# learnedsystems/RMI

Hardware: NVIDIA H100
Metric: RMI build keys/sec (200M uint64, linear,linear 2^20) (higher is better)
Workload: dtype f64

## Files before the change

### rmi_b200/csrc/api.cu

```cuda
#include <algorithm>
#include <fcntl.h>
#include <sys/mman.h>
#include <unistd.h>
#include <atomic>
#include <chrono>
#include <cstdlib>
#include <cmath>
#include <cstdio>
#include <cstring>
#include <memory>
#include <mutex>
#include <string>
#include <vector>

#include "../../include/rmi_b200.h"
#include "kernels.h"
#include "nccl_dl.h"
#include "../../host/cache_fix.hpp"
#include "../../host/artefact_load.hpp"
#include "../../host/codegen.hpp"
#include "../../host/optimizer.hpp"
#include "../../host/slab_layout.hpp"

using namespace rmi;
// ... 573 lines not shown
    rmihost::output_rmi(ns, *r, data_dir, key_type, include_errors != 0, build_time_ns, out_dir, knots ? &cf : nullptr);
    return RMI_OK;
  } catch (const std::exception& e) {
    return fail(RMI_ERR_PANIC, e.what());
  }
}

int rmi_load_rmi(const char* ns, const char* out_dir, const char* data_dir, rmi_result** out, rmi_spline_point** knots,
                 rmi_artefact_info* info) {
  g_last_error.clear();
  if (!ns || !out_dir || !data_dir || !out || !knots || !info) return fail(RMI_ERR_INVALID, "rmi_load_rmi: null argument");
  auto a = std::make_unique<rmihost::LoadedArtefact>();
  try {
    rmihost::load_rmi(ns, out_dir, data_dir, a.get());
  } catch (const rmihost::LoadError& e) {
    return fail(e.code, e.what());
  } catch (const std::exception& e) {
    return fail(RMI_ERR_INVALID, std::string("rmi_load_rmi: ") + e.what());
  }
  rmi_spline_point* pts = nullptr;
  if (!a->knots.empty()) {
    pts = static_cast<rmi_spline_point*>(std::malloc(a->knots.size() * sizeof(rmi_spline_point)));
    if (!pts) return fail(RMI_ERR_INVALID, "rmi_load_rmi: out of host memory");
    for (size_t k = 0; k < a->knots.size(); ++k) { pts[k].key = a->knots[k].first; pts[k].offset = a->knots[k].second; }
  }
  auto box = new ResultBox();
  box->pub = a->r;
  *out = &box->pub;
  *knots = pts;
  info->key_type = a->key_type;
  info->has_errors = a->has_errors ? 1 : 0;
  info->line_size = a->line_size;
  info->num_knots = a->knots.size();
  info->num_data_rows = a->r.num_data_rows;
  info->build_time_ns = a->build_time_ns;
  box->loaded = std::move(a);
  return RMI_OK;
}

int rmi_find_pareto_efficient_configs(const rmi_dataset* const* replicas, int num_replicas, uint64_t restrict_to,
                                      uint32_t flags, rmi_config_stats* out, uint64_t capacity, uint64_t* out_count) {
  g_last_error.clear();
  if (!replicas || num_replicas < 1 || !out_count || (capacity && !out))
    return fail(RMI_ERR_INVALID, "rmi_find_pareto_efficient_configs: bad argument");
  try {
    std::vector<const rmi_dataset*> reps(replicas, replicas + num_replicas);
    std::vector<rmihost::RMIStatistics> front = rmihost::find_pareto_efficient_configs(reps, (size_t)restrict_to, flags, false);
    *out_count = front.size();
    for (size_t i = 0; i < front.size() && i < capacity; ++i) {
      std::snprintf(out[i].models, sizeof out[i].models, "%s", front[i].models.c_str());
      out[i].branching_factor = front[i].branching_factor;
      out[i].average_log2_error = front[i].average_log2_error;
      out[i].max_log2_error = front[i].max_log2_error;
      out[i].size = front[i].size;
    }
    return RMI_OK;
  } catch (const std::exception& e) {
    return fail(RMI_ERR_PANIC, e.what());
  }
}

int rmi_dataset_replicate(const rmi_dataset* src, int device, rmi_dataset** out) {
  g_last_error.clear();
  if (!src || !out) return fail(RMI_ERR_INVALID, "rmi_dataset_replicate: null argument");
  const size_t ksz = src->key_type == RMI_KEY_U32 ? 4 : 8;
  const size_t bytes = ((size_t)src->n * ksz + 15) & ~(size_t)15;
  CUDA_TRY(cudaSetDevice(device));
  void* d = nullptr;
  CUDA_TRY(cudaMalloc(&d, bytes ? bytes : 16));
  cudaError_t e = cudaSuccess;
  if (src->n) {
    if (device != src->device) {
      int can = 0;
      cudaDeviceCanAccessPeer(&can, device, src->device);
      if (can) { cudaError_t pe = cudaDeviceEnablePeerAccess(src->device, 0); if (pe != cudaSuccess) cudaGetLastError(); }
    }
    e = cudaMemcpyPeer(d, device, src->d_keys, src->device, (size_t)src->n * ksz);
    if (e == cudaSuccess) e = cudaDeviceSynchronize();
  }
  if (e != cudaSuccess) { cudaFree(d); return fail(RMI_ERR_CUDA, std::string("rmi_dataset_replicate: ") + cudaGetErrorString(e)); }
  auto* ds = new rmi_dataset();
  ds->d_keys = d; ds->n = src->n; ds->key_type = src->key_type; ds->device = device;
  ds->owned = true; ds->pooled = false; ds->sorted = src->sorted; ds->no_dups = src->no_dups;
  *out = ds;
  return RMI_OK;
}

uint64_t rmi_dataset_len(const rmi_dataset* ds) { return ds ? ds->n : 0; }
int rmi_dataset_key_type(const rmi_dataset* ds) { return ds ? ds->key_type : -1; }
void rmi_dataset_destroy(rmi_dataset* ds) {
  if (!ds) return;
  if (ds->owned && ds->d_keys) {
    cudaSetDevice(ds->device);
    if (ds->pooled) cudaFreeAsync(ds->d_keys, nullptr); else cudaFree(ds->d_keys);
  }
  delete ds;
}

void rmi_result_free(rmi_result* r) { delete reinterpret_cast<ResultBox*>(r); }

}

struct rmi_index {
  const rmi_dataset* ds = nullptr;
  TopTables tables;
  TopModel top;
  int leaf_kind = 0;
  uint64_t N = 0;
  uint64_t n = 0;
  void* d_records = nullptr;
  int num_sms = 0;
  void* d_knots = nullptr;
  uint64_t K = 0;
  uint64_t line_size = 0;
};

namespace {
void index_free_device(rmi_index* idx) {
  idx->tables.free_device();
  cudaFree(idx->d_records);
  cudaFree(idx->d_knots);
}

int index_check_call(const rmi_index* idx, const void* d_queries, uint64_t n, const void* d_out, const char* fn) {
  if (!idx) return fail(RMI_ERR_INVALID, std::string(fn) + ": null index");
  if (n && (!d_queries || !d_out)) return fail(RMI_ERR_INVALID, std::string(fn) + ": null query or output pointer");
  return RMI_OK;
}

int index_launch(const rmi_index* idx, const void* d_queries, uint64_t n, uint64_t* d_out, uint64_t* d_err,
                 uint64_t* d_fallbacks, void* cuda_stream, bool lower_bound) {
  if (n == 0) return RMI_OK;
  const rmi_dataset* ds = idx->ds;
  CUDA_TRY(cudaSetDevice(ds->device));
  Launch L{(cudaStream_t)cuda_stream, idx->num_sms};
  if (idx->d_knots) {
    lookup_bounded_batch(L, idx->top, idx->leaf_kind, idx->d_records, idx->N, idx->d_knots, idx->K, idx->line_size,
                         (const u64*)ds->d_keys, idx->n, (const u64*)d_queries, n, (u64*)d_out, (u64*)d_err,
                         (u64*)d_fallbacks, lower_bound);
    CUDA_TRY(cudaGetLastError());
    return RMI_OK;
  }
  with_key_type(ds->key_type, [&](auto k) {
    using T = decltype(k);
    lookup_batch<T>(L, idx->top, idx->leaf_kind, idx->d_records, idx->N, (const T*)ds->d_keys, idx->n,
                    (const T*)d_queries, n, (u64*)d_out, (u64*)d_err, (u64*)d_fallbacks, lower_bound);
  });
  CUDA_TRY(cudaGetLastError());
  return RMI_OK;
}
int index_check_tables(const rmi_result* r, uint64_t rows, const char* holder, uint64_t keys, const std::string& fn) {
  if (r->num_rmi_rows != rows)
    return fail(RMI_ERR_INVALID, fn + ": the result was trained on " + std::to_string(r->num_rmi_rows) + " keys, " +
                                     holder + std::to_string(rows));
  if (keys == 0 || r->branching_factor == 0) return fail(RMI_ERR_INVALID, fn + ": empty index");
  return RMI_OK;
}

int index_upload(const rmi_result* r, const rmi_dataset* ds, uint64_t n, const rmi_spline_point* knots, uint64_t K,
                 uint64_t line_size, const std::string& fn, rmi_index** out) {
  CUDA_TRY(cudaSetDevice(ds->device));
  DeviceInfo di;
  if (int rc = device_info(ds->device, &di)) return rc;
  auto* idx = new rmi_index();
  idx->ds = ds;
  idx->leaf_kind = (int)r->l1_model_id;
  idx->N = r->branching_factor;
  idx->n = n;
  idx->num_sms = di.num_sms;
  std::vector<char> packed((size_t)idx->N * lookup_record_bytes(idx->leaf_kind));
  pack_leaf_records(idx->leaf_kind, r->l1_params, (const u64*)r->l1_errors, idx->N, packed.data());
  cudaError_t e = idx->tables.upload(*r, nullptr, device_alloc);
  idx->top = idx->tables.given(*r);
  if (e == cudaSuccess) e = cudaMalloc(&idx->d_records, packed.size());
  if (e == cudaSuccess) e = cudaMemcpy(idx->d_records, packed.data(), packed.size(), cudaMemcpyHostToDevice);
  if (e == cudaSuccess && knots) {
    e = cudaMalloc(&idx->d_knots, sizeof(rmi_spline_point) * K);
    if (e == cudaSuccess) e = cudaMemcpy(idx->d_knots, knots, sizeof(rmi_spline_point) * K, cudaMemcpyHostToDevice);
    idx->K = K;
    idx->line_size = line_size;
  }
  if (e == cudaSuccess) e = cudaStreamSynchronize(nullptr);
  if (e != cudaSuccess) {
    index_free_device(idx);
    delete idx;
    return fail(RMI_ERR_CUDA, fn + ": " + cudaGetErrorString(e));
  }
  *out = idx;
  return RMI_OK;
}


}

extern "C" {

int rmi_index_create(const rmi_result* r, const rmi_dataset* ds, rmi_index** out) {
  const std::string fn = "rmi_index_create";
  if (!r || !ds || !out) return fail(RMI_ERR_INVALID, fn + ": null argument");
  if (int rc = check_result(r, true, fn)) return rc;
  if (int rc = index_check_tables(r, ds->n, "the dataset holds ", ds->n, fn)) return rc;
  return index_upload(r, ds, ds->n, nullptr, 0, 0, fn, out);
}

int rmi_index_create_bounded(const rmi_result* r, const rmi_spline_point* knots, uint64_t num_knots,
                             uint64_t line_size, const rmi_dataset* ds, rmi_index** out) {
  const std::string fn = "rmi_index_create_bounded";
  if (!r || !knots || !ds || !out) return fail(RMI_ERR_INVALID, fn + ": null argument");
  if (int rc = check_result(r, true, fn)) return rc;
  if (ds->key_type != RMI_KEY_U64) return fail(RMI_ERR_INVALID, fn + ": Can only construct a bounded RMI on u64 data");
  if (line_size == 0) return fail(RMI_ERR_INVALID, fn + ": line size 0");
  if (num_knots == 0) return fail(RMI_ERR_INVALID, fn + ": no spline knots");
  if (int rc = index_check_tables(r, num_knots, "the spline has ", ds->n, fn)) return rc;
  for (uint64_t i = 0; i < num_knots; ++i) {
    if (knots[i].offset >= ds->n)
      return fail(RMI_ERR_INVALID, fn + ": knot " + std::to_string(i) + " has offset " + std::to_string(knots[i].offset) +
                                       ", the dataset holds " + std::to_string(ds->n) + " keys");
    if (i && !(knots[i - 1].key < knots[i].key && knots[i - 1].offset <= knots[i].offset))
      return fail(RMI_ERR_INVALID, fn + ": knots " + std::to_string(i - 1) + " and " + std::to_string(i) +
                                       " are out of order (keys must increase strictly, offsets must not decrease)");
  }
  return index_upload(r, ds, ds->n, knots, num_knots, line_size, fn, out);
}

void rmi_index_destroy(rmi_index* idx) {
  if (!idx) return;
  cudaSetDevice(idx->ds->device);
  index_free_device(idx);
  delete idx;
}

int rmi_index_predict(const rmi_index* idx, const void* d_queries, uint64_t n, uint64_t* d_pos, uint64_t* d_err,
                      void* cuda_stream) {
  if (int rc = index_check_call(idx, d_queries, n, d_pos, "rmi_index_predict")) return rc;
  return index_launch(idx, d_queries, n, d_pos, d_err, nullptr, cuda_stream, false);
}

int rmi_index_lower_bound(const rmi_index* idx, const void* d_queries, uint64_t n, uint64_t* d_out,
                          uint64_t* d_fallbacks, void* cuda_stream) {
  if (int rc = index_check_call(idx, d_queries, n, d_out, "rmi_index_lower_bound")) return rc;
  return index_launch(idx, d_queries, n, d_out, nullptr, d_fallbacks, cuda_stream, true);
}

int rmi_index_lookup_host(const rmi_index* idx, const void* host_queries, uint64_t n, int lower_bound,
                          uint64_t* host_out, uint64_t* host_err, uint64_t* fallbacks) {
  if (int rc = index_check_call(idx, host_queries, n, host_out, "rmi_index_lookup_host")) return rc;
  if (n == 0) return RMI_OK;
  CUDA_TRY(cudaSetDevice(idx->ds->device));
  const size_t qb = (size_t)n * key_bytes(idx->ds->key_type), ob = (size_t)n * sizeof(uint64_t);
  cudaStream_t st = nullptr;
  char* d = nullptr;
  cudaError_t e = cudaStreamCreateWithFlags(&st, cudaStreamNonBlocking);
  if (e == cudaSuccess) e = cudaMallocAsync((void**)&d, qb + 2 * ob + 8 + 8, st);
  int rc = RMI_OK;
  if (e == cudaSuccess) {
    char* d_q = d;
    uint64_t* d_out = (uint64_t*)(d + ((qb + 7) & ~(size_t)7));
    uint64_t* d_err = d_out + n;
    uint64_t* d_fb = d_err + n;
    e = cudaMemcpyAsync(d_q, host_queries, qb, cudaMemcpyHostToDevice, st);
    if (e == cudaSuccess) e = cudaMemsetAsync(d_fb, 0, sizeof(u64), st);
    if (e == cudaSuccess) {
      rc = lower_bound ? index_launch(idx, d_q, n, d_out, nullptr, d_fb, st, true)
                       : index_launch(idx, d_q, n, d_out, host_err ? d_err : nullptr, nullptr, st, false);
    }
    if (e == cudaSuccess && rc == RMI_OK) e = cudaMemcpyAsync(host_out, d_out, ob, cudaMemcpyDeviceToHost, st);
    if (e == cudaSuccess && rc == RMI_OK && !lower_bound && host_err)
      e = cudaMemcpyAsync(host_err, d_err, ob, cudaMemcpyDeviceToHost, st);
    if (e == cudaSuccess && rc == RMI_OK && lower_bound && fallbacks)
      e = cudaMemcpyAsync(fallbacks, d_fb, sizeof(u64), cudaMemcpyDeviceToHost, st);
    cudaFreeAsync(d, st);
  }
  if (st) {
    cudaError_t es = cudaStreamSynchronize(st);
    if (e == cudaSuccess) e = es;
    cudaStreamDestroy(st);
  }
  if (rc != RMI_OK) return rc;
  if (e != cudaSuccess) return fail(RMI_ERR_CUDA, std::string("rmi_index_lookup_host: ") + cudaGetErrorString(e));
  return RMI_OK;
}

}

namespace {

struct SliceResources {
  int device = -1;
  LeafCopyOut co;
  void release() {
    if (device < 0) return;
    for (int c = 0; c < LEAF_SLICES; ++c) {
      if (co.streams[c]) cudaStreamDestroy(co.streams[c]);
      if (co.ev_kernel[c]) cudaEventDestroy(co.ev_kernel[c]);
      if (co.ev_copied[c]) cudaEventDestroy(co.ev_copied[c]);
    }
    if (co.ev_ready) cudaEventDestroy(co.ev_ready);
    co = LeafCopyOut();
    device = -1;
  }
  LeafCopyOut* get(int dev) {
    if (device == dev) return &co;
    release();
    bool ok = cudaEventCreateWithFlags(&co.ev_ready, cudaEventDisableTiming) == cudaSuccess;
    for (int c = 0; c < LEAF_SLICES && ok; ++c)
      ok = cudaStreamCreateWithFlags(&co.streams[c], cudaStreamNonBlocking) == cudaSuccess &&
           cudaEventCreateWithFlags(&co.ev_kernel[c], cudaEventDisableTiming) == cudaSuccess &&
           cudaEventCreateWithFlags(&co.ev_copied[c], cudaEventDisableTiming) == cudaSuccess;
    device = dev;
    if (!ok) { release(); cudaGetLastError(); return nullptr; }
    return &co;
  }
  ~SliceResources() {}
};
thread_local SliceResources t_slices;

struct BuildContext {
  int device = -1;
  cudaStream_t st = nullptr, side = nullptr;
  cudaEvent_t ev0 = nullptr, ev1 = nullptr, evp[3] = {nullptr, nullptr, nullptr}, ev_fork = nullptr, ev_join = nullptr;
  void release() {
    if (device < 0) return;
    if (st) cudaStreamDestroy(st);
    if (side) cudaStreamDestroy(side);
    for (cudaEvent_t e : {ev0, ev1, evp[0], evp[1], evp[2], ev_fork, ev_join}) if (e) cudaEventDestroy(e);
    *this = BuildContext();
  }
  BuildContext* get(int dev) {
    if (device == dev) return this;
    release();
    int lo_prio = 0, hi_prio = 0;
    cudaDeviceGetStreamPriorityRange(&lo_prio, &hi_prio);
    bool ok = cudaStreamCreateWithFlags(&st, cudaStreamNonBlocking) == cudaSuccess &&
              cudaEventCreate(&ev0) == cudaSuccess && cudaEventCreate(&ev1) == cudaSuccess &&
              cudaEventCreate(&evp[0]) == cudaSuccess && cudaEventCreate(&evp[1]) == cudaSuccess &&
              cudaEventCreate(&evp[2]) == cudaSuccess &&
              cudaEventCreateWithFlags(&ev_fork, cudaEventDisableTiming) == cudaSuccess &&
              cudaEventCreateWithFlags(&ev_join, cudaEventDisableTiming) == cudaSuccess;
    if (ok && cudaStreamCreateWithPriority(&side, cudaStreamNonBlocking, hi_prio) != cudaSuccess) { side = nullptr; cudaGetLastError(); }
    device = dev;
    if (!ok) { release(); cudaGetLastError(); return nullptr; }
    return this;
  }
};
thread_local BuildContext t_build_ctx;

struct Arena {
  cudaStream_t st;
  std::vector<void*> ptrs;
  cudaError_t err = cudaSuccess;
  explicit Arena(cudaStream_t s) : st(s) {}
  template <class P> P* get(size_t count) {
    void* p = nullptr;
    cudaError_t e = cudaMallocAsync(&p, std::max<size_t>(count * sizeof(P), 16), st);
    if (e != cudaSuccess) { err = e; return nullptr; }
    ptrs.push_back(p);
    return (P*)p;
  }
  ~Arena() { for (void* p : ptrs) cudaFreeAsync(p, st); }
};

template <class T> inline double host_as_float(T k) { return (double)k; }
inline uint64_t host_scale(uint64_t off, double sf, bool use_sf) { return use_sf ? (uint64_t)((double)off * sf) : off; }

template <class T>
unsigned host_exact_top(const rmi_dataset* ds, int kind, uint64_t N, double* out_f) {
  const uint64_t n = ds->n;
  const T* d_keys = (const T*)ds->d_keys;
  const double sf = (double)N / (double)n;
  const bool use_sf = std::fabs(sf - 1.0) > DBL_EPSILON;
  uint64_t i0 = 0, i1 = n;
  bool repeat = true;
  if (kind == M_ROBUST_LINEAR) {
    uint64_t bnd = (uint64_t)((double)n * 0.0001);
    if (bnd < 1) bnd = 1;
    if (!(bnd * 2 + 1 < n)) return ST_ROBUST_TOO_SMALL;
    i0 = bnd; i1 = n - bnd; repeat = false;
  }
  const size_t PIECE = ((size_t)64 << 20) / sizeof(T);
  T* stage[2] = {(T*)g_pinned.get(PIECE * sizeof(T)), (T*)g_pinned.get(PIECE * sizeof(T))};
  cudaStream_t cs = nullptr;
  cudaEvent_t ev[2] = {nullptr, nullptr};
  bool ok = stage[0] && stage[1] && cudaStreamCreateWithFlags(&cs, cudaStreamNonBlocking) == cudaSuccess &&
            cudaEventCreateWithFlags(&ev[0], cudaEventDisableTiming) == cudaSuccess &&
            cudaEventCreateWithFlags(&ev[1], cudaEventDisableTiming) == cudaSuccess;
  unsigned status = 0;
  if (ok) {
    const int passes = kind == M_NORMAL ? 2 : 1;
    double mean_x = 0.0, mean_y = 0.0, c = 0.0, m2 = 0.0;
    uint64_t cnt = 0;
    double nmean = 0.0, nstd = 0.0;
    const double nf = (double)n;
    T last_key = T();
    uint64_t last_F = 0;
    for (int pass = 0; pass < passes && ok; ++pass) {
      auto issue = [&](uint64_t piece) {
        const uint64_t a = piece * PIECE, b = std::min<uint64_t>(n, a + PIECE);
        cudaMemcpyAsync(stage[piece & 1], d_keys + a, (b - a) * sizeof(T), cudaMemcpyDeviceToHost, cs);
        cudaEventRecord(ev[piece & 1], cs);
      };
      const uint64_t npieces = (n + PIECE - 1) / PIECE;
      if (npieces) issue(0);
      uint64_t F = 0;
      T prev = T();
      for (uint64_t piece = 0; piece < npieces && ok; ++piece) {
        if (cudaEventSynchronize(ev[piece & 1]) != cudaSuccess) { ok = false; break; }
        if (piece + 1 < npieces) issue(piece + 1);
        const T* kb = stage[piece & 1];
        const uint64_t a = piece * PIECE, b = std::min<uint64_t>(n, a + PIECE);
        for (uint64_t i = a; i < b; ++i) {
          const T k = kb[i - a];
          if (i == 0 || k != prev) F = i;
          prev = k;
          if (kind == M_NORMAL) {
            const double x = host_as_float(k);
            if (pass == 0) nmean = nmean + x / nf;
            else { const double d = x - nmean; nstd = nstd + d * d; }
          } else if (i >= i0 && i < i1) {
            const double x = host_as_float(k), y = (double)host_scale(F, sf, use_sf);
            cnt += 1;
            const double dx = x - mean_x;
            const double cf = (double)cnt;
            mean_x = mean_x + dx / cf;
            mean_y = mean_y + (y - mean_y) / cf;
            c = c + dx * (y - mean_y);
            const double dx2 = x - mean_x;
            m2 = m2 + dx * dx2;
          }
        }
        if (b == n && n > 0) { last_key = prev; last_F = F; }
      }
      if (!ok) break;
      if (n > 0) {
        const double x = host_as_float(last_key);
        if (kind == M_NORMAL) {
          if (pass == 0) nmean = nmean + x / nf;
          else { const double d = x - nmean; nstd = nstd + d * d; }
        } else if (repeat) {
          const double y = (double)host_scale(last_F, sf, use_sf);
          cnt += 1;
          const double dx = x - mean_x;
          const double cf = (double)cnt;
          mean_x = mean_x + dx / cf;
          mean_y = mean_y + (y - mean_y) / cf;
          c = c + dx * (y - mean_y);
          const double dx2 = x - mean_x;
          m2 = m2 + dx * dx2;
        }
      }
    }
    if (ok) {
      if (kind == M_NORMAL) {
        out_f[0] = nmean;
        out_f[1] = std::sqrt(nstd / nf);
        out_f[2] = n > 0 ? std::fmax(-INFINITY, (double)host_scale(last_F, sf, use_sf)) : -INFINITY;
      } else {
        double alpha, beta;
        if (cnt == 0) { alpha = 0.0; beta = 0.0; }
        else if (cnt == 1) { alpha = mean_y; beta = 0.0; }
        else {
          const double nm1 = (double)(cnt - 1);
          const double cov = c / nm1, var = m2 / nm1;
          if (!(var >= 0.0)) { status |= ST_NEG_VARIANCE; alpha = 0.0; beta = 0.0; }
          else if (var == 0.0) { alpha = mean_y; beta = 0.0; }
          else { beta = cov / var; alpha = mean_y - beta * mean_x; }
        }
        out_f[0] = alpha; out_f[1] = beta;
      }
    }
  }
  if (cs) { cudaStreamSynchronize(cs); cudaStreamDestroy(cs); }
  for (cudaEvent_t e : ev) if (e) cudaEventDestroy(e);
  g_pinned.put(stage[0]); g_pinned.put(stage[1]);
  if (!ok) return 0x80000000u;
  return status;
}
inline bool serial_top_kind(int kind) {
  return kind == M_LINEAR || kind == M_ROBUST_LINEAR || kind == M_LOGLINEAR || kind == M_NORMAL;
}
inline bool host_exact_kind(int kind) { return kind == M_LINEAR || kind == M_ROBUST_LINEAR || kind == M_NORMAL; }
constexpr uint64_t HOST_EXACT_MIN = (uint64_t)1 << 20;

template <class T>
int train_typed(const rmi_dataset* ds, const ModelName& top, const ModelName& leaf, uint64_t N, uint32_t flags,
                const double* l0_over, uint32_t n_over, rmi_result** out) {
  auto t_start = std::chrono::steady_clock::now();
  const uint64_t n = ds->n;
  const T* keys = (const T*)ds->d_keys;
  CUDA_TRY(cudaSetDevice(ds->device));
  DeviceInfo di;
  if (int rc = device_info(ds->device, &di)) return rc;

  BuildContext* bc = t_build_ctx.get(ds->device);
  if (!bc) return fail(RMI_ERR_CUDA, "could not create the build's CUDA streams / events");
  cudaStream_t st = bc->st;
  cudaEvent_t ev0 = bc->ev0, ev1 = bc->ev1, *evp = bc->evp;
  int rc = RMI_OK;
  auto box = new ResultBox();
  {
    Arena A(st);
    Launch L{st, di.num_sms};
    L.side = bc->side; L.ev_fork = bc->ev_fork; L.ev_join = bc->ev_join;
    L.d_long = A.get<u32>(LONG_LEAF_CAP + 1);
    const int ppm = leaf_params_per_model(leaf.kind);
    TopModel* d_top = A.get<TopModel>(1);
    BuildAux* d_aux = A.get<BuildAux>(1);
    u64* d_S = A.get<u64>(N + 1);
    double* d_params = A.get<double>(N * ppm);
    u64* d_errors = A.get<u64>(N);
    u64* d_counts = A.get<u64>(N);
    void* d_scratch = A.get<char>(top_scratch_bytes(N));
    void* d_stats = A.get<char>(stats_scratch_bytes(N));
    T* d_sample = !l0_over && top_fit_writes_sample(top.kind, (flags & RMI_FLAG_TOP_FIT_EXACT) != 0)
                      ? bounds_sample_at<T>(A.get<char>(bounds_sample_bytes(n, sizeof(T)))) : nullptr;
    TopTables tables;
    tables.allocate(top, n, N, [&](size_t bytes) -> void* { return A.get<char>(bytes); });
    const bool stats_only = (flags & RMI_FLAG_STATS_ONLY) != 0;
    const bool want_counts = !stats_only && (flags & RMI_FLAG_LEAF_COUNTS) != 0;
    const bool host_ok = reserve_result(box, &tables, N, ppm, !stats_only, want_counts);
    if (A.err != cudaSuccess) {
      rc = fail(RMI_ERR_CUDA, std::string("scratch allocation: ") + cudaGetErrorString(A.err));
    } else if (!host_ok) {
      rc = fail(RMI_ERR_CUDA, kPinnedFailed);
    } else {
      TopModel h_top = tables.initial(top, l0_over, n_over);
      cudaEventRecord(ev0, st);
      unsigned host_status = 0;
      bool exact = (flags & RMI_FLAG_TOP_FIT_EXACT) != 0;
      bool host_top = false;
      if (exact && !l0_over && host_exact_kind(top.kind) && n >= HOST_EXACT_MIN) {
        cudaEventSynchronize(ev0);
        unsigned hs = host_exact_top<T>(ds, top.kind, N, h_top.f);
        if (hs == 0x80000000u) rc = fail(RMI_ERR_CUDA, "exact top fit: copying the keys back to the host failed");
        else { host_status |= hs; host_top = true; }
      }
      cudaMemcpyAsync(d_top, &h_top, sizeof(h_top), cudaMemcpyHostToDevice, st);
      cudaMemsetAsync(d_aux, 0, sizeof(BuildAux), st);
      bool leaf_results_copied = false;
      if (!l0_over && !host_top && rc == RMI_OK)
        host_status |= fit_top_model<T>(L, keys, n, top.kind, top.table_bits, N, exact, d_top, d_aux, d_scratch, tables.t32,
                                        tables.pivots, tables.radix_index, d_sample);
      cudaEventRecord(evp[0], st);
      if (host_status == 0 && rc == RMI_OK) {
        compute_leaf_bounds<T>(L, keys, n, top.kind, d_top, N, d_S, d_aux, l0_over == nullptr, d_sample);
        cudaEventRecord(evp[1], st);
        {
          Shard<T> whole = whole_array<T>(n);
          whole.no_dups = ds->no_dups ? 1 : 0;
          LeafCopyOut* co = stats_only ? nullptr : t_slices.get(ds->device);
          if (co) {
            co->h_params = box->l1_params.data(); co->h_errors = reinterpret_cast<u64*>(box->l1_errors.data());
            co->h_counts = want_counts ? reinterpret_cast<u64*>(box->l1_counts.data()) : nullptr;
            co->used = 0;
            L.copy = co;
            leaf_results_copied = true;
          }
          fit_leaves<T>(L, keys, whole, leaf.kind, N, d_S, d_aux, d_params, d_errors, d_counts);
        }
        cudaEventRecord(evp[2], st);
        leaf_statistics(L, n, N, d_errors, d_counts, d_aux, d_stats);
      } else {
        cudaEventRecord(evp[1], st);
        cudaEventRecord(evp[2], st);
      }
      cudaEventRecord(ev1, st);
      leaf_copy_join(L);
      const bool fitted = host_status == 0;
      copy_result_to_host(box, fitted ? &tables : nullptr, d_aux, d_top,
                          fitted && !stats_only && !leaf_results_copied ? d_params : nullptr, d_errors,
                          want_counts ? d_counts : nullptr, st);
      cudaError_t e = cudaStreamSynchronize(st);
      if (rc != RMI_OK) {
      } else if (e != cudaSuccess) {
        rc = fail(RMI_ERR_CUDA, std::string("rmi_train: ") + cudaGetErrorString(e));
      } else if (host_status | result_aux(box).status) {
        rc = fail(RMI_ERR_PANIC, status_text(host_status | result_aux(box).status));
      } else {
        fill_result(box, top, leaf, tables, n, N);
        rmi_result& R = box->pub;
        R.device_time_ns = elapsed_ns(ev0, ev1);
        cudaEvent_t seq[5] = {ev0, evp[0], evp[1], evp[2], ev1};
        for (int q = 0; q < 4; ++q) R.phase_device_ns[q] = elapsed_ns(seq[q], seq[q + 1]);
        R.top_fit_exact = (exact && !l0_over && serial_top_kind(top.kind)) ? 1 : 0;
      }
    }
  }
  cudaStreamSynchronize(st);
  if (rc != RMI_OK) { delete box; return rc; }
  box->pub.build_time_ns =
      (uint64_t)std::chrono::duration_cast<std::chrono::nanoseconds>(std::chrono::steady_clock::now() - t_start).count();
  *out = &box->pub;
  return RMI_OK;
}

template <class T>
int train_batch_typed(const rmi_dataset* ds, const ModelName& top, const std::vector<const ModelName*>& leaves, uint64_t N,
                      uint32_t flags, rmi_result** out) {
  auto t_start = std::chrono::steady_clock::now();
  const uint64_t n = ds->n;
  const T* keys = (const T*)ds->d_keys;
  CUDA_TRY(cudaSetDevice(ds->device));
  DeviceInfo di;
  if (int rc = device_info(ds->device, &di)) return rc;
  BuildContext* bc = t_build_ctx.get(ds->device);
  if (!bc) return fail(RMI_ERR_CUDA, "could not create the build's CUDA streams / events");
  cudaStream_t st = bc->st;
  const size_t K = leaves.size();
  std::vector<ResultBox*> boxes(K, nullptr);
  int rc = RMI_OK;
  {
    Arena A(st);
    Launch L{st, di.num_sms};
    L.side = bc->side; L.ev_fork = bc->ev_fork; L.ev_join = bc->ev_join;
    L.d_long = A.get<u32>(LONG_LEAF_CAP + 1);
    int max_ppm = 2;
    for (auto* lf : leaves) max_ppm = std::max(max_ppm, leaf_params_per_model(lf->kind));
    TopModel* d_top = A.get<TopModel>(1);
    BuildAux* d_aux0 = A.get<BuildAux>(1);
    BuildAux* d_auxk = A.get<BuildAux>(K);
    u64* d_S = A.get<u64>(N + 1);
    double* d_params = A.get<double>(N * max_ppm);
    u64* d_errors = A.get<u64>(N);
    u64* d_counts = A.get<u64>(N);
    void* d_scratch = A.get<char>(top_scratch_bytes(N));
    void* d_stats = A.get<char>(stats_scratch_bytes(N));
    T* d_sample = top_fit_writes_sample(top.kind, (flags & RMI_FLAG_TOP_FIT_EXACT) != 0)
                      ? bounds_sample_at<T>(A.get<char>(bounds_sample_bytes(n, sizeof(T)))) : nullptr;
    TopTables tables;
    tables.allocate(top, n, N, [&](size_t bytes) -> void* { return A.get<char>(bytes); });
    bool host_ok = true;
    for (size_t k = 0; k < K; ++k) {
      boxes[k] = new ResultBox();
      host_ok = host_ok && reserve_result(boxes[k], nullptr, N, 0, false, false);
    }
    if (A.err != cudaSuccess) rc = fail(RMI_ERR_CUDA, std::string("scratch allocation: ") + cudaGetErrorString(A.err));
    else if (!host_ok) rc = fail(RMI_ERR_CUDA, kPinnedFailed);
    else {
      const TopModel h_top = tables.initial(top);
      cudaEventRecord(bc->ev0, st);
      cudaMemcpyAsync(d_top, &h_top, sizeof(h_top), cudaMemcpyHostToDevice, st);
      cudaMemsetAsync(d_aux0, 0, sizeof(BuildAux), st);
      const bool exact = (flags & RMI_FLAG_TOP_FIT_EXACT) != 0;
      unsigned host_status = fit_top_model<T>(L, keys, n, top.kind, top.table_bits, N, exact, d_top, d_aux0, d_scratch,
                                              tables.t32, tables.pivots, tables.radix_index, d_sample);
      if (host_status == 0) {
        compute_leaf_bounds<T>(L, keys, n, top.kind, d_top, N, d_S, d_aux0, true, d_sample);
        Shard<T> whole = whole_array<T>(n);
        whole.no_dups = ds->no_dups ? 1 : 0;
        for (size_t k = 0; k < K; ++k) {
          BuildAux* d_aux = d_auxk + k;
          cudaMemcpyAsync(d_aux, d_aux0, sizeof(BuildAux), cudaMemcpyDeviceToDevice, st);
          fit_leaves<T>(L, keys, whole, leaves[k]->kind, N, d_S, d_aux, d_params, d_errors, d_counts);
          leaf_statistics(L, n, N, d_errors, d_counts, d_aux, d_stats);
          copy_result_to_host(boxes[k], nullptr, d_aux, d_top, nullptr, nullptr, nullptr, st);
        }
      }
      cudaEventRecord(bc->ev1, st);
      cudaError_t e = cudaStreamSynchronize(st);
      if (e != cudaSuccess) rc = fail(RMI_ERR_CUDA, std::string("rmi_train_stats_batch: ") + cudaGetErrorString(e));
      else if (host_status) rc = fail(RMI_ERR_PANIC, status_text(host_status));
      else {
        float ms = 0.f;
        cudaEventElapsedTime(&ms, bc->ev0, bc->ev1);
        for (size_t k = 0; k < K && rc == RMI_OK; ++k) {
          const unsigned status = result_aux(boxes[k]).status;
          if (status) { rc = fail(RMI_ERR_PANIC, std::string(top.name) + "," + leaves[k]->name + ": " + status_text(status)); break; }
          fill_result(boxes[k], top, *leaves[k], tables, n, N);
          boxes[k]->pub.device_time_ns = (uint64_t)((double)ms * 1e6 / (double)K);
          boxes[k]->pub.top_fit_exact = exact && serial_top_kind(top.kind) ? 1 : 0;
        }
      }
    }
  }
  cudaStreamSynchronize(st);
  if (rc != RMI_OK) { for (auto* b : boxes) delete b; return rc; }
  const uint64_t wall = (uint64_t)std::chrono::duration_cast<std::chrono::nanoseconds>(std::chrono::steady_clock::now() - t_start).count();
  for (size_t k = 0; k < K; ++k) { boxes[k]->pub.build_time_ns = wall / K; out[k] = &boxes[k]->pub; }
  return RMI_OK;
}

int train_entry(const rmi_dataset* ds, const char* model_spec, uint64_t N, uint32_t flags, const double* l0_over,
                uint32_t n_over, rmi_result** out) {
  g_last_error.clear();
  if (!ds || !model_spec || !out) return fail(RMI_ERR_INVALID, "rmi_train: null argument");
  const ModelName *top = nullptr, *leaf = nullptr;
  if (int rc = parse_two_layer(model_spec, &top, &leaf)) return rc;
  if (int rc = check_build(ds->n, N, ds->sorted)) return rc;
  if (l0_over && (top->fparams == 0 || n_over != (uint32_t)top->fparams))
    return fail(RMI_ERR_INVALID, "rmi_train_with_top: top model has no float parameters or wrong count");
  return with_key_type(ds->key_type, [&](auto k) {
    return train_typed<decltype(k)>(ds, *top, *leaf, N, flags, l0_over, n_over, out);
  });
}

constexpr unsigned kEvaluateStatus = ST_NOT_SORTED | ST_NON_MONOTONE;

void fill_given_result(ResultBox* box, const rmi_result* r, const ModelName& top, const ModelName& leaf,
                       const TopTables& tables, uint64_t n, bool stats_only) {
  const uint64_t N = r->branching_factor;
  if (!stats_only) memcpy(box->l1_params.data(), r->l1_params, sizeof(double) * N * leaf_params_per_model(leaf.kind));
  if (tables.t32_len) memcpy(box->table32.data(), r->l0_table32, sizeof(u32) * tables.t32_len);
  if (tables.ri_len) memcpy(box->arr1.data(), r->l0_array1, sizeof(u64) * tables.ri_len);
  if (tables.hist_bins) memcpy(box->arr2.data(), r->l0_array2, sizeof(u64) * tables.hist_bins);
  fill_result(box, top, leaf, tables, n, N);
  rmi_result& R = box->pub;
  R.l0_num_fparams = r->l0_num_fparams;
  R.l0_num_iparams = r->l0_num_iparams;
  R.top_fit_exact = r->top_fit_exact;
}

template <class T>
int evaluate_typed(const rmi_dataset* ds, const rmi_result* r, const ModelName& top, const ModelName& leaf, uint32_t flags,
                   rmi_result** out) {
  auto t_start = std::chrono::steady_clock::now();
  const uint64_t n = ds->n, N = r->branching_factor;
  const T* keys = (const T*)ds->d_keys;
  CUDA_TRY(cudaSetDevice(ds->device));
  DeviceInfo di;
  if (int rc = device_info(ds->device, &di)) return rc;
  BuildContext* bc = t_build_ctx.get(ds->device);
  if (!bc) return fail(RMI_ERR_CUDA, "could not create the build's CUDA streams / events");
  cudaStream_t st = bc->st;
  cudaEvent_t ev0 = bc->ev0, ev1 = bc->ev1, *evp = bc->evp;
  const int ppm = leaf_params_per_model(leaf.kind);
  const bool stats_only = (flags & RMI_FLAG_STATS_ONLY) != 0;
  const bool want_counts = !stats_only && (flags & RMI_FLAG_LEAF_COUNTS) != 0;
  int rc = RMI_OK;
  auto box = new ResultBox();
  {
    Arena A(st);
    Launch L{st, di.num_sms};
    TopModel* d_top = A.get<TopModel>(1);
    BuildAux* d_aux = A.get<BuildAux>(1);
    u64* d_S = A.get<u64>(N + 1);
    double* d_params = A.get<double>(N * ppm);
    u64* d_errors = A.get<u64>(N);
    u64* d_counts = A.get<u64>(N);
    u64* d_scratch = A.get<u64>(2 * N);
    void* d_stats = A.get<char>(stats_scratch_bytes(N));
    TopTables tables;
    cudaEventRecord(ev0, st);
    const cudaError_t te = tables.upload(*r, st, [&](size_t bytes) -> void* { return A.get<char>(bytes); });
    const bool host_ok = reserve_result(box, &tables, N, ppm, !stats_only, want_counts);
    if (A.err != cudaSuccess) {
      rc = fail(RMI_ERR_CUDA, std::string("scratch allocation: ") + cudaGetErrorString(A.err));
    } else if (te != cudaSuccess) {
      rc = fail(RMI_ERR_CUDA, std::string("rmi_evaluate: ") + cudaGetErrorString(te));
    } else if (!host_ok) {
      rc = fail(RMI_ERR_CUDA, kPinnedFailed);
    } else {
      const TopModel h_top = tables.given(*r);
      cudaMemcpyAsync(d_top, &h_top, sizeof(h_top), cudaMemcpyHostToDevice, st);
      cudaMemcpyAsync(d_params, r->l1_params, sizeof(double) * N * ppm, cudaMemcpyHostToDevice, st);
      cudaMemsetAsync(d_aux, 0, sizeof(BuildAux), st);
      cudaEventRecord(evp[0], st);
      compute_leaf_bounds<T>(L, keys, n, top.kind, d_top, N, d_S, d_aux, false, nullptr);
      cudaEventRecord(evp[1], st);
      evaluate_leaves<T>(L, keys, n, ds->no_dups, leaf.kind, N, d_S, d_params, d_scratch, d_errors, d_counts);
      cudaEventRecord(evp[2], st);
      leaf_statistics(L, n, N, d_errors, d_counts, d_aux, d_stats);
      cudaEventRecord(ev1, st);
      copy_result_to_host(box, nullptr, d_aux, d_top, nullptr, nullptr, nullptr, st);
      if (!stats_only) {
        cudaMemcpyAsync(box->l1_errors.data(), d_errors, sizeof(u64) * N, cudaMemcpyDeviceToHost, st);
        if (want_counts) cudaMemcpyAsync(box->l1_counts.data(), d_counts, sizeof(u64) * N, cudaMemcpyDeviceToHost, st);
      }
      cudaError_t e = cudaStreamSynchronize(st);
      const unsigned status = e == cudaSuccess ? result_aux(box).status & kEvaluateStatus : 0;
      if (e != cudaSuccess) {
        rc = fail(RMI_ERR_CUDA, std::string("rmi_evaluate: ") + cudaGetErrorString(e));
      } else if (status) {
        rc = fail(RMI_ERR_PANIC, status_text(status));
      } else {
        fill_given_result(box, r, top, leaf, tables, n, stats_only);
        rmi_result& R = box->pub;
        R.device_time_ns = elapsed_ns(ev0, ev1);
        cudaEvent_t seq[5] = {ev0, evp[0], evp[1], evp[2], ev1};
        for (int q = 0; q < 4; ++q) R.phase_device_ns[q] = elapsed_ns(seq[q], seq[q + 1]);
      }
    }
  }
  cudaStreamSynchronize(st);
  if (rc != RMI_OK) { delete box; return rc; }
  box->pub.build_time_ns =
      (uint64_t)std::chrono::duration_cast<std::chrono::nanoseconds>(std::chrono::steady_clock::now() - t_start).count();
  *out = &box->pub;
  return RMI_OK;
}

}

extern "C" {

void rmi_thread_release(void) {
  t_build_ctx.release();
  t_slices.release();
}

int rmi_train(const rmi_dataset* ds, const char* model_spec, uint64_t branch_factor, uint32_t flags, rmi_result** out) {
  return train_entry(ds, model_spec, branch_factor, flags, nullptr, 0, out);
}
int rmi_train_stats_batch(const rmi_dataset* ds, const char* top_model, const char* const* leaf_models, int num_leaf_models,
                          uint64_t branch_factor, uint32_t flags, rmi_result** out) {
  g_last_error.clear();
  if (!ds || !top_model || !leaf_models || num_leaf_models < 1 || !out) return fail(RMI_ERR_INVALID, "rmi_train_stats_batch: bad argument");
  const ModelName* top = nullptr;
  if (int rc = find_layer(top_model, true, &top)) return rc;
  std::vector<const ModelName*> leaves(num_leaf_models);
  for (int k = 0; k < num_leaf_models; ++k) {
    if (int rc = find_layer(leaf_models[k] ? leaf_models[k] : "(null)", false, &leaves[k])) return rc;
    if (int rc = check_leaf(leaves[k])) return rc;
  }
  if (int rc = check_build(ds->n, branch_factor, ds->sorted)) return rc;
  return with_key_type(ds->key_type, [&](auto k) {
    return train_batch_typed<decltype(k)>(ds, *top, leaves, branch_factor, flags, out);
  });
}
int rmi_train_with_top(const rmi_dataset* ds, const char* model_spec, uint64_t branch_factor, uint32_t flags,
                       const double* l0_fparams, uint32_t n_fparams, rmi_result** out) {
  if (!l0_fparams) return fail(RMI_ERR_INVALID, "rmi_train_with_top: null parameters");
  return train_entry(ds, model_spec, branch_factor, flags, l0_fparams, n_fparams, out);
}

int rmi_evaluate(const rmi_dataset* ds, const rmi_result* r, uint32_t flags, rmi_result** out) {
  g_last_error.clear();
  const std::string fn = "rmi_evaluate";
  if (!ds || !r || !out) return fail(RMI_ERR_INVALID, fn + ": null argument");
  const ModelName *top = nullptr, *leaf = nullptr;
  if (int rc = check_result(r, false, fn, &top, &leaf)) return rc;
  if (int rc = check_build(ds->n, r->branching_factor, ds->sorted)) return rc;
  return with_key_type(ds->key_type, [&](auto k) { return evaluate_typed<decltype(k)>(ds, r, *top, *leaf, flags, out); });
}

int rmi_cache_fix_device(const rmi_dataset* ds, uint64_t line_size, rmi_spline_point** out_points, uint64_t* out_count,
                         rmi_cache_fix_stats* stats) {
  g_last_error.clear();
  const std::string fn = "rmi_cache_fix_device";
  if (!ds || !out_points || !out_count) return fail(RMI_ERR_INVALID, fn + ": null argument");
  if (ds->key_type != RMI_KEY_U64) return fail(RMI_ERR_INVALID, fn + ": Can only construct a bounded RMI on u64 data");
  const uint64_t n = ds->n;
  if (!(n > line_size)) return fail(RMI_ERR_PANIC, "Cannot apply a cachefix with fewer items than the line size");
  if (line_size == 0) return fail(RMI_ERR_PANIC, "attempt to divide by zero");
  if (!ds->sorted) return fail(RMI_ERR_PANIC, "keys are not sorted in ascending order");
  CUDA_TRY(cudaSetDevice(ds->device));
  DeviceInfo di;
  if (int rc = device_info(ds->device, &di)) return rc;
  BuildContext* bc = t_build_ctx.get(ds->device);
  if (!bc) return fail(RMI_ERR_CUDA, fn + ": could not create the CUDA stream");
  cudaStream_t st = bc->st;
  const u64* keys = (const u64*)ds->d_keys;
  uint64_t first = 0;
  CUDA_TRY(cudaMemcpyAsync(&first, keys, sizeof(u64), cudaMemcpyDeviceToHost, st));
  CUDA_TRY(cudaStreamSynchronize(st));
  if (first == 0) return fail(RMI_ERR_PANIC, "When source x is 18446744073709551615, cannot set dest x to 0");

  const u64 chunk = CACHEFIX_CHUNK, nch = (n + chunk - 1) / chunk;
  u64 h_stats[CF_NUM_STATS] = {};
  rmi_spline_point* host = nullptr;
  u64 total = 0;
  cudaError_t e = cudaSuccess;
  {
    Arena A(st);
    CacheFixScratch s;
    s.targets = A.get<u64>(nch * CACHEFIX_TARGETS);
    s.spec_count = A.get<u64>(nch);
    s.spec_exit = A.get<u64>(nch);
    s.stitch_exit = A.get<u64>(nch);
    s.stitch_ok = A.get<u32>(nch);
    s.entry = A.get<u64>(nch);
    s.count = A.get<u64>(nch);
    s.offsets = A.get<u64>(nch + 1);
    s.last_knot = A.get<u64>(2);
    s.stats = A.get<u64>(CF_NUM_STATS);
    e = A.err;
    if (e == cudaSuccess) e = cudaMemsetAsync(s.stats, 0, sizeof(u64) * CF_NUM_STATS, st);
    Launch L{st, di.num_sms};
    if (e == cudaSuccess) {
      cache_fix_scan(L, keys, n, line_size, chunk, s);
      e = cudaGetLastError();
    }
    if (e == cudaSuccess) e = cudaMemcpyAsync(&total, s.offsets + nch, sizeof(u64), cudaMemcpyDeviceToHost, st);
    if (e == cudaSuccess) e = cudaStreamSynchronize(st);
    ++total;
    u64* d_out = e == cudaSuccess ? A.get<u64>(2 * total) : nullptr;
    if (e == cudaSuccess) e = A.err;
    if (e == cudaSuccess) {
      cache_fix_emit(L, keys, n, line_size, chunk, s, d_out);
      e = cudaGetLastError();
    }
    if (e == cudaSuccess) e = cudaMemcpyAsync(h_stats, s.stats, sizeof h_stats, cudaMemcpyDeviceToHost, st);
    if (e == cudaSuccess) {
      host = static_cast<rmi_spline_point*>(std::malloc(total * sizeof(rmi_spline_point)));
      if (!host) return fail(RMI_ERR_INVALID, fn + ": out of host memory");
      e = cudaMemcpyAsync(host, d_out, total * sizeof(rmi_spline_point), cudaMemcpyDeviceToHost, st);
    }
    if (e == cudaSuccess) e = cudaStreamSynchronize(st);
  }
  if (e == cudaSuccess) e = cudaStreamSynchronize(st);
  if (e != cudaSuccess) {
    std::free(host);
    return fail(RMI_ERR_CUDA, fn + ": " + cudaGetErrorString(e));
  }
  *out_points = host;
  *out_count = total;
  if (stats) {
    stats->chunk_keys = chunk;
    stats->chunks = nch;
    stats->points = h_stats[CF_STAT_POINTS];
    stats->stitch_segments = h_stats[CF_STAT_STITCH_SEGMENTS];
    stats->fallback_points = h_stats[CF_STAT_FALLBACK_POINTS];
    stats->evaluations = h_stats[CF_STAT_EVALS];
  }
  return RMI_OK;
}

}

using rmihost::bits_from_key;
using rmihost::key_from_bits;
using rmihost::SlabLayout;

struct rmi_shard_build {
  const rmi_dataset* ds = nullptr;
  SlabLayout lay;
  uint64_t halo_capacity = 0;
  rmi_shard_buffers buf{};
  const ModelName* top = nullptr;
  const ModelName* leaf = nullptr;
  uint64_t N = 0;
  uint64_t halo = 0;
  cudaStream_t st = nullptr;
  int num_sms = 0;
  TopModel* d_top = nullptr;
  BuildAux* d_aux = nullptr;
  void* d_scratch = nullptr;
  void* d_stats = nullptr;
  unsigned host_status = 0;
  std::chrono::steady_clock::time_point t_start;
  cudaStream_t side = nullptr;
  cudaEvent_t ev_fork = nullptr, ev_join = nullptr;
  u32* d_long = nullptr;
  cudaEvent_t ev_begin[RMI_NUM_PHASES] = {};
  cudaEvent_t ev_end[RMI_NUM_PHASES] = {};
  bool ran[RMI_NUM_PHASES] = {};
  int world = 0, rank = 0, r_last = 0;
  u64* d_bases = nullptr;
  u64* d_off = nullptr;
  u64* h_off = nullptr;
  void* d_parts = nullptr;
  unsigned* d_flags_mine = nullptr;
  unsigned* d_flags_all = nullptr;
  unsigned* h_flags_all = nullptr;
  bool gather_mode = false;
  const LeafCopyOut* leaf_copy = nullptr;
  u64 leaf_lo = 0, leaf_hi = 0;
  TopTables tables;
  cudaEvent_t ev_off = nullptr, ev_t0 = nullptr, ev_t1 = nullptr;
};

struct rmi_shard_comm {
  ncclComm_t comm = nullptr;
  int world = 0, rank = 0, device = 0;
  bool single_node = false;
  uint32_t uid_hash = 0;
  int shm_gen = 0;
  unsigned char* shm = nullptr;
  size_t shm_half = 0;
  int parity = 0;
  cudaStream_t copy_stream = nullptr;
  cudaEvent_t ev_leaf_done = nullptr, ev_copy_done = nullptr;
  unsigned* d_token = nullptr;
};

namespace {

template <class T> Shard<T> shard_of(const SlabLayout& lay, uint64_t n_local, uint64_t n_avail) {
  Shard<T> s;
  s.base = lay.base;
  s.n_global = lay.n_global;
  s.n_local = n_local;
  s.n_avail = n_avail;
  s.has_prev = lay.has_prev;
  s.is_last = lay.is_last;
  s.prev_key = key_from_bits<T>(lay.prev_key_bits);
  s.prev_F = lay.prev_F;
  s.no_dups = lay.no_dups ? 1 : 0;
  return s;
}

template <class T> int shard_ends_typed(const rmi_dataset* ds, rmi_shard_ends* out) {
  out->n_local = ds->n;
  out->no_dups = ds->no_dups ? 1 : 0;
  out->first_key_bits = out->last_key_bits = out->last_run_start = 0;
  if (ds->n == 0) return RMI_OK;
  const T* keys = (const T*)ds->d_keys;
  T first, last;
  CUDA_TRY(cudaMemcpy(&first, keys, sizeof(T), cudaMemcpyDeviceToHost));
  CUDA_TRY(cudaMemcpy(&last, keys + (ds->n - 1), sizeof(T), cudaMemcpyDeviceToHost));
  out->first_key_bits = bits_from_key<T>(first);
  out->last_key_bits = bits_from_key<T>(last);
  uint64_t lo = 0, hi = ds->n - 1;
  while (lo < hi) {
    uint64_t mid = lo + (hi - lo) / 2;
    T v;
    CUDA_TRY(cudaMemcpy(&v, keys + mid, sizeof(T), cudaMemcpyDeviceToHost));
    if (v == last) hi = mid; else lo = mid + 1;
  }
  out->last_run_start = lo;
  return RMI_OK;
}

template <class T> int shard_phase_typed(rmi_shard_build* b, int phase) {
  const T* keys = (const T*)b->ds->d_keys;
  Shard<T> sh = shard_of<T>(b->lay, b->ds->n, b->ds->n + b->halo);
  Launch L{b->st, b->num_sms};
  L.side = b->side; L.ev_fork = b->ev_fork; L.ev_join = b->ev_join; L.d_long = b->d_long;
  const int ppm = leaf_params_per_model(b->leaf->kind);
  if (phase >= 0 && phase < RMI_NUM_PHASES) { cudaEventRecord(b->ev_begin[phase], b->st); b->ran[phase] = true; }
  if (phase == RMI_PHASE_TOP_LOCAL) {
    b->t_start = std::chrono::steady_clock::now();
    b->host_status = 0;
    for (int q = 1; q < RMI_NUM_PHASES; ++q) b->ran[q] = false;
  }
  const T first_key = key_from_bits<T>(b->lay.first_key_bits), last_key = key_from_bits<T>(b->lay.last_key_bits);
  const TopTables& tt = b->tables;
  switch (phase) {
    case RMI_PHASE_TOP_LOCAL:
      cudaMemsetAsync(b->d_aux, 0, sizeof(BuildAux), b->st);
      {
        const TopModel h = tt.initial(*b->top);
        cudaMemcpyAsync(b->d_top, &h, sizeof(h), cudaMemcpyHostToDevice, b->st);
      }
      if (b->top->kind == M_HISTOGRAM && (tt.hist_bins == 0 || tt.hist_ipb < 1)) b->host_status |= ST_HIST_BINS;
      b->host_status |= shard_top_local<T>(L, keys, sh, b->top->kind, b->N, b->lay.pivot_x, b->lay.pivot_y, first_key,
                                           last_key, b->d_scratch, (double*)b->buf.sums);
      if ((b->top->kind == M_RADIX_TABLE || b->top->kind == M_HISTOGRAM) && b->host_status == 0)
        shard_table_local<T>(L, keys, sh, b->top->kind, b->top->table_bits, b->N, first_key, last_key, b->d_aux, tt.t32,
                             tt.pivots, tt.hist_bins, tt.hist_ipb);
      break;
    case RMI_PHASE_TOP_MID:
      shard_top_mid<T>(L, keys, sh, b->top->kind, b->N, first_key, last_key, b->d_scratch, (double*)b->buf.sums, b->d_aux);
      break;
    case RMI_PHASE_TOP_FINISH:
      shard_top_finish<T>(L, sh, b->top->kind, b->N, b->lay.pivot_x, b->lay.pivot_y, (const double*)b->buf.sums,
                          first_key, last_key, b->lay.last_F, b->d_scratch, b->d_top, b->d_aux);
      if (b->top->kind == M_RADIX_TABLE && b->host_status == 0) shard_table_decode(L, b->top->table_bits, tt.t32);
      if (b->top->kind == M_HISTOGRAM && b->host_status == 0) hist_radix_index(L, tt.pivots, tt.hist_bins, tt.radix_index);
      break;
    case RMI_PHASE_BOUNDS:
      shard_bounds<T>(L, keys, sh, b->top->kind, b->d_top, b->N, (u64*)b->buf.S, b->d_aux);
      break;
    case RMI_PHASE_SPLIT:
      shard_split<T>(L, keys, sh, b->top->kind, b->d_top, b->N, (const u64*)b->buf.S, b->d_aux);
      break;
    case RMI_PHASE_LEAF:
      if (!b->gather_mode) {
        cudaMemsetAsync(b->buf.params, 0, sizeof(double) * b->N * ppm, b->st);
        cudaMemsetAsync(b->buf.errors, 0, sizeof(u64) * b->N, b->st);
        cudaMemsetAsync(b->buf.counts, 0, sizeof(u64) * b->N, b->st);
      }
      L.copy = b->leaf_copy; L.leaf_lo = b->leaf_lo; L.leaf_hi = b->leaf_hi;
      fit_leaves<T>(L, keys, sh, b->leaf->kind, b->N, (const u64*)b->buf.S, b->d_aux, (double*)b->buf.params,
                    (u64*)b->buf.errors, (u64*)b->buf.counts);
      L.copy = nullptr; L.leaf_lo = L.leaf_hi = 0;
      shard_copy_status(L, b->d_aux, (unsigned*)b->buf.status);
      break;
    case RMI_PHASE_STATS:
      leaf_statistics(L, b->lay.n_global, b->N, (const u64*)b->buf.errors, (const u64*)b->buf.counts, b->d_aux, b->d_stats);
      break;
    default:
      return fail(RMI_ERR_INVALID, "rmi_shard_phase: unknown phase");
  }
  if (phase >= 0 && phase < RMI_NUM_PHASES) cudaEventRecord(b->ev_end[phase], b->st);
  cudaError_t e = cudaGetLastError();
  if (e != cudaSuccess) return fail(RMI_ERR_CUDA, std::string("rmi_shard_phase: ") + cudaGetErrorString(e));
  return RMI_OK;
}

int check_slabs(const std::string& fn, const rmi_dataset* local, const rmi_shard_ends* ends_all, int world, int rank,
                uint64_t* base, uint64_t* total) {
  if (world < 1 || world > SHARD_ROUTE_MAX - 1 || rank < 0 || rank >= world)
    return fail(RMI_ERR_INVALID, fn + ": bad world or rank (0 <= rank < world <= 63)");
  if (ends_all[rank].n_local != local->n)
    return fail(RMI_ERR_INVALID, fn + ": ends_all[" + std::to_string(rank) + "] describes " +
                                     std::to_string(ends_all[rank].n_local) + " keys, the local dataset holds " +
                                     std::to_string(local->n));
// ... 1107 lines not shown
```

Baseline: 94.26 billion.

## Persist build scratch across calls, merge init uploads, prioritize slice streams

Result: faster. 101.5 billion, median of 6 (+7.7%).

```diff
diff --git a/rmi_b200/csrc/api.cu b/rmi_b200/csrc/api.cu
--- a/rmi_b200/csrc/api.cu
+++ b/rmi_b200/csrc/api.cu
@@ -899,9 +899,11 @@
   LeafCopyOut* get(int dev) {
     if (device == dev) return &co;
     release();
+    int least = 0, greatest = 0;
+    cudaDeviceGetStreamPriorityRange(&least, &greatest);
     bool ok = cudaEventCreateWithFlags(&co.ev_ready, cudaEventDisableTiming) == cudaSuccess;
     for (int c = 0; c < LEAF_SLICES && ok; ++c)
-      ok = cudaStreamCreateWithFlags(&co.streams[c], cudaStreamNonBlocking) == cudaSuccess &&
+      ok = cudaStreamCreateWithPriority(&co.streams[c], cudaStreamNonBlocking, std::min(least, greatest + 1 + c)) == cudaSuccess &&
            cudaEventCreateWithFlags(&co.ev_kernel[c], cudaEventDisableTiming) == cudaSuccess &&
            cudaEventCreateWithFlags(&co.ev_copied[c], cudaEventDisableTiming) == cudaSuccess;
     device = dev;
@@ -916,8 +918,15 @@
   int device = -1;
   cudaStream_t st = nullptr, side = nullptr;
   cudaEvent_t ev0 = nullptr, ev1 = nullptr, evp[3] = {nullptr, nullptr, nullptr}, ev_fork = nullptr, ev_join = nullptr;
+  char* scratch = nullptr;
+  size_t scratch_cap = 0;
+  char* h_init = nullptr;
+  static constexpr size_t kInitBytes = sizeof(TopModel) + sizeof(BuildAux);
+  static constexpr size_t kScratchKeepMax = (size_t)1 << 30;
   void release() {
     if (device < 0) return;
+    if (scratch) cudaFree(scratch);
+    if (h_init) cudaFreeHost(h_init);
     if (st) cudaStreamDestroy(st);
     if (side) cudaStreamDestroy(side);
     for (cudaEvent_t e : {ev0, ev1, evp[0], evp[1], evp[2], ev_fork, ev_join}) if (e) cudaEventDestroy(e);
@@ -933,14 +942,51 @@
               cudaEventCreate(&evp[0]) == cudaSuccess && cudaEventCreate(&evp[1]) == cudaSuccess &&
               cudaEventCreate(&evp[2]) == cudaSuccess &&
               cudaEventCreateWithFlags(&ev_fork, cudaEventDisableTiming) == cudaSuccess &&
-              cudaEventCreateWithFlags(&ev_join, cudaEventDisableTiming) == cudaSuccess;
+              cudaEventCreateWithFlags(&ev_join, cudaEventDisableTiming) == cudaSuccess &&
+              cudaMallocHost((void**)&h_init, kInitBytes) == cudaSuccess;
     if (ok && cudaStreamCreateWithPriority(&side, cudaStreamNonBlocking, hi_prio) != cudaSuccess) { side = nullptr; cudaGetLastError(); }
     device = dev;
     if (!ok) { release(); cudaGetLastError(); return nullptr; }
     return this;
   }
+  void upload_init(void* d_init, const TopModel& top) {
+    memcpy(h_init, &top, sizeof(TopModel));
+    memset(h_init + sizeof(TopModel), 0, sizeof(BuildAux));
+    cudaMemcpyAsync(d_init, h_init, kInitBytes, cudaMemcpyHostToDevice, st);
+  }
+  void grow_scratch(size_t bytes) {
+    if (bytes <= scratch_cap || bytes > kScratchKeepMax) return;
+    if (scratch) cudaFreeAsync(scratch, st);
+    scratch = nullptr;
+    scratch_cap = 0;
+    if (cudaMallocAsync((void**)&scratch, bytes, st) == cudaSuccess) scratch_cap = bytes;
+    else { scratch = nullptr; cudaGetLastError(); }
+  }
 };
 thread_local BuildContext t_build_ctx;
+static_assert(sizeof(TopModel) % alignof(BuildAux) == 0, "the BuildAux after a TopModel in one upload must be aligned");
+
+struct BuildScratch {
+  BuildContext* bc;
+  size_t used = 0;
+  std::vector<void*> extra;
+  cudaError_t err = cudaSuccess;
+  explicit BuildScratch(BuildContext* c) : bc(c) {}
+  template <class P> P* get(size_t count) {
+    const size_t bytes = (std::max<size_t>(count * sizeof(P), 16) + 255) & ~(size_t)255;
+    used += bytes;
+    if (used <= bc->scratch_cap) return (P*)(bc->scratch + used - bytes);
+    void* p = nullptr;
+    cudaError_t e = cudaMallocAsync(&p, bytes, bc->st);
+    if (e != cudaSuccess) { err = e; return nullptr; }
+    extra.push_back(p);
+    return (P*)p;
+  }
+  ~BuildScratch() {
+    for (void* p : extra) cudaFreeAsync(p, bc->st);
+    if (err == cudaSuccess) bc->grow_scratch(used);
+  }
+};
 
 struct Arena {
   cudaStream_t st;
@@ -1095,13 +1141,14 @@
   int rc = RMI_OK;
   auto box = new ResultBox();
   {
-    Arena A(st);
+    BuildScratch A(bc);
     Launch L{st, di.num_sms};
     L.side = bc->side; L.ev_fork = bc->ev_fork; L.ev_join = bc->ev_join;
     L.d_long = A.get<u32>(LONG_LEAF_CAP + 1);
     const int ppm = leaf_params_per_model(leaf.kind);
-    TopModel* d_top = A.get<TopModel>(1);
-    BuildAux* d_aux = A.get<BuildAux>(1);
+    char* d_init = A.get<char>(BuildContext::kInitBytes);
+    TopModel* d_top = reinterpret_cast<TopModel*>(d_init);
+    BuildAux* d_aux = reinterpret_cast<BuildAux*>(d_init + sizeof(TopModel));
     u64* d_S = A.get<u64>(N + 1);
     double* d_params = A.get<double>(N * ppm);
     u64* d_errors = A.get<u64>(N);
@@ -1131,8 +1178,7 @@
         if (hs == 0x80000000u) rc = fail(RMI_ERR_CUDA, "exact top fit: copying the keys back to the host failed");
         else { host_status |= hs; host_top = true; }
       }
-      cudaMemcpyAsync(d_top, &h_top, sizeof(h_top), cudaMemcpyHostToDevice, st);
-      cudaMemsetAsync(d_aux, 0, sizeof(BuildAux), st);
+      bc->upload_init(d_init, h_top);
       bool leaf_results_copied = false;
       if (!l0_over && !host_top && rc == RMI_OK)
         host_status |= fit_top_model<T>(L, keys, n, top.kind, top.table_bits, N, exact, d_top, d_aux, d_scratch, tables.t32,
@@ -1182,8 +1228,7 @@
       }
     }
   }
-  cudaStreamSynchronize(st);
-  if (rc != RMI_OK) { delete box; return rc; }
+  if (rc != RMI_OK) { cudaStreamSynchronize(st); delete box; return rc; }
   box->pub.build_time_ns =
       (uint64_t)std::chrono::duration_cast<std::chrono::nanoseconds>(std::chrono::steady_clock::now() - t_start).count();
   *out = &box->pub;
@@ -1206,14 +1251,15 @@
   std::vector<ResultBox*> boxes(K, nullptr);
   int rc = RMI_OK;
   {
-    Arena A(st);
+    BuildScratch A(bc);
     Launch L{st, di.num_sms};
     L.side = bc->side; L.ev_fork = bc->ev_fork; L.ev_join = bc->ev_join;
     L.d_long = A.get<u32>(LONG_LEAF_CAP + 1);
     int max_ppm = 2;
     for (auto* lf : leaves) max_ppm = std::max(max_ppm, leaf_params_per_model(lf->kind));
-    TopModel* d_top = A.get<TopModel>(1);
-    BuildAux* d_aux0 = A.get<BuildAux>(1);
+    char* d_init = A.get<char>(BuildContext::kInitBytes);
+    TopModel* d_top = reinterpret_cast<TopModel*>(d_init);
+    BuildAux* d_aux0 = reinterpret_cast<BuildAux*>(d_init + sizeof(TopModel));
     BuildAux* d_auxk = A.get<BuildAux>(K);
     u64* d_S = A.get<u64>(N + 1);
     double* d_params = A.get<double>(N * max_ppm);
@@ -1235,8 +1281,7 @@
     else {
       const TopModel h_top = tables.initial(top);
       cudaEventRecord(bc->ev0, st);
-      cudaMemcpyAsync(d_top, &h_top, sizeof(h_top), cudaMemcpyHostToDevice, st);
-      cudaMemsetAsync(d_aux0, 0, sizeof(BuildAux), st);
+      bc->upload_init(d_init, h_top);
       const bool exact = (flags & RMI_FLAG_TOP_FIT_EXACT) != 0;
       unsigned host_status = fit_top_model<T>(L, keys, n, top.kind, top.table_bits, N, exact, d_top, d_aux0, d_scratch,
                                               tables.t32, tables.pivots, tables.radix_index, d_sample);
@@ -1269,8 +1314,7 @@
       }
     }
   }
-  cudaStreamSynchronize(st);
-  if (rc != RMI_OK) { for (auto* b : boxes) delete b; return rc; }
+  if (rc != RMI_OK) { cudaStreamSynchronize(st); for (auto* b : boxes) delete b; return rc; }
   const uint64_t wall = (uint64_t)std::chrono::duration_cast<std::chrono::nanoseconds>(std::chrono::steady_clock::now() - t_start).count();
   for (size_t k = 0; k < K; ++k) { boxes[k]->pub.build_time_ns = wall / K; out[k] = &boxes[k]->pub; }
   return RMI_OK;
@@ -1325,10 +1369,11 @@
   int rc = RMI_OK;
   auto box = new ResultBox();
   {
-    Arena A(st);
+    BuildScratch A(bc);
     Launch L{st, di.num_sms};
-    TopModel* d_top = A.get<TopModel>(1);
-    BuildAux* d_aux = A.get<BuildAux>(1);
+    char* d_init = A.get<char>(BuildContext::kInitBytes);
+    TopModel* d_top = reinterpret_cast<TopModel*>(d_init);
+    BuildAux* d_aux = reinterpret_cast<BuildAux*>(d_init + sizeof(TopModel));
     u64* d_S = A.get<u64>(N + 1);
     double* d_params = A.get<double>(N * ppm);
     u64* d_errors = A.get<u64>(N);
@@ -1347,9 +1392,8 @@
       rc = fail(RMI_ERR_CUDA, kPinnedFailed);
     } else {
       const TopModel h_top = tables.given(*r);
-      cudaMemcpyAsync(d_top, &h_top, sizeof(h_top), cudaMemcpyHostToDevice, st);
+      bc->upload_init(d_init, h_top);
       cudaMemcpyAsync(d_params, r->l1_params, sizeof(double) * N * ppm, cudaMemcpyHostToDevice, st);
-      cudaMemsetAsync(d_aux, 0, sizeof(BuildAux), st);
       cudaEventRecord(evp[0], st);
       compute_leaf_bounds<T>(L, keys, n, top.kind, d_top, N, d_S, d_aux, false, nullptr);
       cudaEventRecord(evp[1], st);
@@ -1377,8 +1421,7 @@
       }
     }
   }
-  cudaStreamSynchronize(st);
-  if (rc != RMI_OK) { delete box; return rc; }
+  if (rc != RMI_OK) { cudaStreamSynchronize(st); delete box; return rc; }
   box->pub.build_time_ns =
       (uint64_t)std::chrono::duration_cast<std::chrono::nanoseconds>(std::chrono::steady_clock::now() - t_start).count();
   *out = &box->pub;
```
